# Anima-Lab/MaskDiT

Hardware: AMD Instinct MI355X
Metric: training img/sec MaskDiT-XL/2 256 mask=0.5 bs=1024 (higher is better)
Workload: dtype bf16; 1 GPU; DiT-XL/2 ImageNet256-latent [32x32x4], mask_ratio=0.5, mae_loss_coef=0.1, sample(moments)+class-dropout+fwd+bwd+grad-allreduce+AdamW+EMA, random-init (de-zeroed) weights; global_batch=1024, per_gpu_batch=1024, micro_batch=1024, accum=1, parallelism=dp1

## Files before the change

maskdit_amd/csrc/attention.hip:

```cpp
#include "common.h"
#include <type_traits>
#include "../../include/maskdit_hip.h"

template <int HD>
struct AttnCfg {
  static constexpr int HDK = (HD + 31) / 32 * 32;
  static constexpr int HDN = (HD + 15) / 16 * 16;
  static constexpr int KSTEPS = HDK / 32;
  static constexpr int NFRAG = HDN / 16;
  static constexpr int CH = HD / 8;
  static constexpr int PITCH_CH = (HDK / 8) | 1;
  static constexpr int PITCH = PITCH_CH * 16;
  static constexpr int TILE_BYTES = 64 * PITCH;
};

template <int HD> struct AttnRow {
  static constexpr int NFRAG = AttnCfg<HD>::NFRAG;
  static constexpr int NP = (NFRAG / 2 < HD / 32) ? NFRAG / 2 : HD / 32;
  static constexpr int NT = NFRAG - 2 * NP;
  uint4 pr[NP > 0 ? NP : 1];
  uint2 tl[NT > 0 ? NT : 1];
};
__device__ __forceinline__ unsigned attn_pack2(float a, float b) {
  bf16x2 t;
// ... 683 lines not shown
          for (int qi = 0; qi < QF; ++qi) s[qi][f] = mfma16(kfr, qf[qi][ks], s[qi][f]);
        }
      }
      bf16x8 pf[QF][KB / 32];
      if (kb + KB > Lv) {
#pragma unroll
        for (int qi = 0; qi < QF; ++qi)
#pragma unroll
          for (int f = 0; f < KB / 16; ++f)
#pragma unroll
            for (int r = 0; r < 4; ++r) s[qi][f][r] = (kb + 16 * f + 4 * g + r < Lv) ? s[qi][f][r] : -1e30f;
      }
#pragma unroll
      for (int qi = 0; qi < QF; ++qi) {
        float mx = -1e30f;
#pragma unroll
        for (int f = 0; f < KB / 16; ++f)
#pragma unroll
          for (int r = 0; r < 4; ++r) mx = fmaxf(mx, s[qi][f][r]);
        mx = group_max(mx);
        const float m_new = fmaxf(m_run[qi], mx * scale_log2e);
        const float alpha = fast_exp2(m_run[qi] - m_new);
        float psum = 0.f;
#pragma unroll
        for (int f = 0; f < KB / 16; ++f)
#pragma unroll
          for (int r = 0; r < 4; ++r) {
            const float pv = fast_exp2(__builtin_fmaf(s[qi][f][r], scale_log2e, -m_new));
            s[qi][f][r] = pv;
            psum += pv;
          }
        l_run[qi] = l_run[qi] * alpha + psum;
        m_run[qi] = m_new;
#pragma unroll
        for (int f = 0; f < C::NFRAG; ++f)
#pragma unroll
          for (int r = 0; r < 4; ++r) o[qi][f][r] *= alpha;
#pragma unroll
        for (int ks = 0; ks < KB / 32; ++ks) pf[qi][ks] = pack_pair(s[qi][2 * ks], s[qi][2 * ks + 1]);
      }
#pragma unroll
      for (int ks = 0; ks < KB / 32; ++ks)
#pragma unroll
        for (int f = 0; f < C::NFRAG; ++f) {
          const bf16x8 vfr = sp_frag_cols<HD, L>(Vs, kb + 32 * ks, f, i16, g);
#pragma unroll
          for (int qi = 0; qi < QF; ++qi) o[qi][f] = mfma16(vfr, pf[qi][ks], o[qi][f]);
        }
    }
#pragma unroll
    for (int qi = 0; qi < QF; ++qi) {
      const int q = wave * 16 * KF + 16 * (qp + qi) + i16;
      const float l_tot = group_sum(l_run[qi]);
      const float inv = 1.f / l_tot;
      bf16* orow = out + ((long)b * L + q) * D + h * HD;
      AttnRow<HD> orw;
      attn_pack_row<HD>(orw, o[qi], inv);
      attn_store_row<HD>(orow, g, orw);
      if (g == 0) lse[((long)b * H + h) * L + q] = m_run[qi] + log2f(l_tot);
    }
  }
}

__device__ __forceinline__ void sp_item_coords(int item, int B, int H, int& b, int& h) {
  const int full = (B >> 3) << 3;
  int sid;
  if (item < full * H) {
    const int xcd = item & 7, k = item >> 3;
    const int grp = k / H;
    sid = (grp * 8 + xcd) * H + (k - grp * H);
  } else {
    sid = item;
  }
  b = sid / H;
  h = sid - b * H;
}

#define SP_LDS_BARRIER()                                 \
  {                                                      \
    asm volatile("s_waitcnt lgkmcnt(0)" ::: "memory");   \
    __builtin_amdgcn_s_barrier();                        \
    asm volatile("" ::: "memory");                       \
  }
template <int HD, int KF, int OCC>
__global__ __launch_bounds__(512, OCC) void attn_bwd_sp_kernel(const bf16* __restrict__ qkv, const bf16* __restrict__ out,
                                                              const bf16* __restrict__ dout, const float* __restrict__ lse,
                                                              float* __restrict__ delta, bf16* __restrict__ dqkv, int H,
                                                              float scale, float scale_log2e, int Lv, int B, int dbg) {
  using C = SpCfg<HD>;
  constexpr int L = 128 * KF;
  constexpr int TILE = L * C::PITCH;
  __shared__ __attribute__((aligned(16))) char smem[4 * TILE + 2 * L * 4 + 64];
  char* Qs = smem;
  char* Ks = smem + TILE;
  char* Vs = smem + 2 * TILE;
  char* dOs = smem + 3 * TILE;
  float* lse_s = (float*)(smem + 4 * TILE);
  float* del_s = lse_s + L;
  const int tid = threadIdx.x, lane = tid & 63, wave = tid >> 6;
  const int i16 = lane & 15, g = lane >> 4;
  const int D = H * HD;
  const long ld = 3L * D;
  const int nitems = B * H;

  SpRegs<HD, L> r0, r1, r2, r3;
  bf16x8 of[KF][C::KSTEPS], dof[KF][C::KSTEPS];
  float lse_r = 0.f;
  auto fetch = [&](int item) {
    int b, h;
    sp_item_coords(item, B, H, b, h);
    const bf16* base = qkv + (long)b * L * ld + h * HD;
    const bf16* dobase = dout + (long)b * L * D + h * HD;
    const bf16* obase = out + (long)b * L * D + h * HD;
    sp_load_nb<HD, L>(r0, base, ld, tid);
    sp_load_nb<HD, L>(r1, base + D, ld, tid);
    sp_load_nb<HD, L>(r2, base + 2 * D, ld, tid);
    sp_load_nb<HD, L>(r3, dobase, D, tid);
    lse_r = lse[((long)b * H + h) * L + (tid & (L - 1))];
#pragma unroll
    for (int qi = 0; qi < KF; ++qi) {
      const int q = wave * 16 * KF + 16 * qi + i16;
#pragma unroll
      for (int s = 0; s < C::KSTEPS; ++s) {
        const int d = min(32 * s + 8 * g, HD - 8);
        of[qi][s] = *(const bf16x8*)(obase + (long)q * D + d);
        dof[qi][s] = *(const bf16x8*)(dobase + (long)q * D + d);
      }
    }
  };

  auto stage = [&](int it) {
    int b, h;
    sp_item_coords(it, B, H, b, h);
    const long bh = (long)b * H + h;
    sp_store<HD, L>(r0, Qs, tid);
    sp_store<HD, L>(r1, Ks, tid);
    sp_store<HD, L>(r2, Vs, tid);
    sp_store<HD, L>(r3, dOs, tid);
    if (tid < L) lse_s[tid] = lse_r;
#pragma unroll
    for (int qi = 0; qi < KF; ++qi) {
      const int q = wave * 16 * KF + 16 * qi + i16;
      float dl = 0.f;
#pragma unroll
      for (int s = 0; s < C::KSTEPS; ++s) {
        float part = 0.f;
#pragma unroll
        for (int e = 0; e < 8; ++e) part += bf2f(dof[qi][s][e]) * bf2f(of[qi][s][e]);
        dl += (32 * s + 8 * g < HD) ? part : 0.f;
      }
      dl = group_sum(dl);
      if (g == 0) {
        del_s[q] = dl * scale;
        delta[bh * L + q] = dl;
      }
    }
  };

  int item = blockIdx.x;
  if (item >= nitems) return;
  fetch(item);
  stage(item);
  for (;;) {
    int b, h;
    sp_item_coords(item, B, H, b, h);
    SP_LDS_BARRIER()
    const bool has_next = OCC == 2 && item + (int)gridDim.x < nitems;
    if (has_next && !MDT_EXP(dbg & 2)) fetch(item + gridDim.x);
    __builtin_amdgcn_sched_barrier(0);

#pragma unroll 1
    for (int ki = 0; ki < (MDT_EXP(dbg & 4) ? 0 : KF); ++ki) {
      const int k0 = wave * 16 * KF + 16 * ki;
      bf16x8 kf[C::KSTEPS], vf[C::KSTEPS];
#pragma unroll
      for (int ks = 0; ks < C::KSTEPS; ++ks) {
        kf[ks] = sp_frag_rows<HD, L>(Ks, k0 + i16, ks, g);
        vf[ks] = sp_frag_rows<HD, L>(Vs, k0 + i16, ks, g);
      }
      f32x4 dk[C::NFRAG], dv[C::NFRAG];
#pragma unroll
      for (int f = 0; f < C::NFRAG; ++f) {
        dk[f] = (f32x4){0.f, 0.f, 0.f, 0.f};
        dv[f] = (f32x4){0.f, 0.f, 0.f, 0.f};
      }
      const bool key_ok = (k0 + i16) < Lv;
#pragma unroll 1
      for (int qb = 0; qb < L; qb += 64) {
        f32x4 pm[4], ds[4];
#pragma unroll
        for (int f = 0; f < 4; ++f) {
          f32x4 s = (f32x4){0.f, 0.f, 0.f, 0.f}, dp = (f32x4){0.f, 0.f, 0.f, 0.f};
#pragma unroll
          for (int ks = 0; ks < C::KSTEPS; ++ks) {
            s = mfma16(sp_frag_rows<HD, L>(Qs, qb + 16 * f + i16, ks, g), kf[ks], s);
            dp = mfma16(sp_frag_rows<HD, L>(dOs, qb + 16 * f + i16, ks, g), vf[ks], dp);
          }
          const f32x4 ls = *(const f32x4*)(lse_s + qb + 16 * f + 4 * g);
          const f32x4 dl = *(const f32x4*)(del_s + qb + 16 * f + 4 * g);
#pragma unroll
          for (int r = 0; r < 4; ++r) {
            const float pv = fast_exp2(__builtin_fmaf(s[r], scale_log2e, -ls[r]));
            pm[f][r] = pv;
            ds[f][r] = pv * __builtin_fmaf(dp[r], scale, -dl[r]);
          }
        }
#pragma unroll
        for (int ks = 0; ks < 2; ++ks) {
          const bf16x8 pf = pack_pair(pm[2 * ks], pm[2 * ks + 1]);
          const bf16x8 dsf = pack_pair(ds[2 * ks], ds[2 * ks + 1]);
#pragma unroll
          for (int f = 0; f < C::NFRAG; ++f) {
            dv[f] = mfma16(sp_frag_cols<HD, L>(dOs, qb + 32 * ks, f, i16, g), pf, dv[f]);
            dk[f] = mfma16(sp_frag_cols<HD, L>(Qs, qb + 32 * ks, f, i16, g), dsf, dk[f]);
          }
        }
      }
      bf16* drow = dqkv + ((long)b * L + k0 + i16) * ld + h * HD;
      AttnRow<HD> krw, vrw;
      if (!key_ok) {
#pragma unroll
        for (int f = 0; f < C::NFRAG; ++f) dk[f] = dv[f] = (f32x4){0.f, 0.f, 0.f, 0.f};
      }
      attn_pack_row<HD>(krw, dk);
      attn_pack_row<HD>(vrw, dv);
      if (!MDT_EXP(dbg & 1)) {
        attn_store_row<HD>(drow + D, g, krw);
        attn_store_row<HD>(drow + 2 * D, g, vrw);
      }
    }

#pragma unroll 1
    for (int qi = 0; qi < (MDT_EXP(dbg & 8) ? 0 : KF); ++qi) {
      const int q = wave * 16 * KF + 16 * qi + i16;
      bf16x8 qf[C::KSTEPS], dqo[C::KSTEPS];
#pragma unroll
      for (int ks = 0; ks < C::KSTEPS; ++ks) {
        qf[ks] = sp_frag_rows<HD, L>(Qs, q, ks, g);
        dqo[ks] = sp_frag_rows<HD, L>(dOs, q, ks, g);
      }
      const float my_lse = lse_s[q], dl = del_s[q];
      f32x4 dq[C::NFRAG];
#pragma unroll
      for (int f = 0; f < C::NFRAG; ++f) dq[f] = (f32x4){0.f, 0.f, 0.f, 0.f};
#pragma unroll 1
      for (int kb = 0; kb < L; kb += 64) {
        f32x4 ds[4];
#pragma unroll
        for (int f = 0; f < 4; ++f) {
          f32x4 s = (f32x4){0.f, 0.f, 0.f, 0.f}, dp = (f32x4){0.f, 0.f, 0.f, 0.f};
#pragma unroll
          for (int ks = 0; ks < C::KSTEPS; ++ks) {
            s = mfma16(sp_frag_rows<HD, L>(Ks, kb + 16 * f + i16, ks, g), qf[ks], s);
            dp = mfma16(sp_frag_rows<HD, L>(Vs, kb + 16 * f + i16, ks, g), dqo[ks], dp);
          }
#pragma unroll
          for (int r = 0; r < 4; ++r) {
            const float pv = fast_exp2(__builtin_fmaf(s[r], scale_log2e, -my_lse));
            ds[f][r] = pv * __builtin_fmaf(dp[r], scale, -dl);
          }
        }
        if (kb + 64 > Lv) {
#pragma unroll
          for (int f = 0; f < 4; ++f)
#pragma unroll
            for (int r = 0; r < 4; ++r) ds[f][r] = (kb + 16 * f + 4 * g + r < Lv) ? ds[f][r] : 0.f;
        }
#pragma unroll
        for (int ks = 0; ks < 2; ++ks) {
          const bf16x8 dsf = pack_pair(ds[2 * ks], ds[2 * ks + 1]);
#pragma unroll
          for (int f = 0; f < C::NFRAG; ++f) dq[f] = mfma16(sp_frag_cols<HD, L>(Ks, kb + 32 * ks, f, i16, g), dsf, dq[f]);
        }
      }
      bf16* drow = dqkv + ((long)b * L + q) * ld + h * HD;
      AttnRow<HD> qrw;
      attn_pack_row<HD>(qrw, dq);
      if (!MDT_EXP(dbg & 1)) attn_store_row<HD>(drow, g, qrw);
    }
    if (!has_next) break;
    SP_LDS_BARRIER()
    item += gridDim.x;
    stage(item);
  }
}

template <int HD>
__device__ __forceinline__ void attn_bwd_item_math(const char* Qs, const char* Ks, const char* Vs, const char* dOs,
                                                   const float* lse_s, const float* del_s, bf16* dbase, long ld, int D,
                                                   int wave, int i16, int g, int Lv, float scale, float scale_log2e,
                                                   AttnRow<HD>& q_cur, const AttnRow<HD>& q_prev) {
  using C = SpCfg<HD>;
  constexpr int L = 128;
  AttnRow<HD> k_keep, v_keep;
  {
    const int k0 = wave * 16;
    bf16x8 kf[C::KSTEPS], vf[C::KSTEPS];
#pragma unroll
    for (int ks = 0; ks < C::KSTEPS; ++ks) {
      kf[ks] = sp_frag_rows<HD, L>(Ks, k0 + i16, ks, g);
      vf[ks] = sp_frag_rows<HD, L>(Vs, k0 + i16, ks, g);
    }
    f32x4 dk[C::NFRAG], dv[C::NFRAG];
#pragma unroll
    for (int f = 0; f < C::NFRAG; ++f) {
      dk[f] = (f32x4){0.f, 0.f, 0.f, 0.f};
      dv[f] = (f32x4){0.f, 0.f, 0.f, 0.f};
    }
    const bool key_ok = (k0 + i16) < Lv;
#pragma unroll 1
    for (int qb = 0; qb < L; qb += 64) {
      f32x4 pm[4], ds[4];
#pragma unroll
      for (int f = 0; f < 4; ++f) {
        f32x4 s = (f32x4){0.f, 0.f, 0.f, 0.f}, dp = (f32x4){0.f, 0.f, 0.f, 0.f};
#pragma unroll
        for (int ks = 0; ks < C::KSTEPS; ++ks) {
          s = mfma16(sp_frag_rows<HD, L>(Qs, qb + 16 * f + i16, ks, g), kf[ks], s);
          dp = mfma16(sp_frag_rows<HD, L>(dOs, qb + 16 * f + i16, ks, g), vf[ks], dp);
        }
        const f32x4 ls = *(const f32x4*)(lse_s + qb + 16 * f + 4 * g);
        const f32x4 dl = *(const f32x4*)(del_s + qb + 16 * f + 4 * g);
#pragma unroll
        for (int r = 0; r < 4; ++r) {
          const float pv = fast_exp2(__builtin_fmaf(s[r], scale_log2e, -ls[r]));
          pm[f][r] = pv;
          ds[f][r] = pv * __builtin_fmaf(dp[r], scale, -dl[r]);
        }
      }
#pragma unroll
      for (int ks = 0; ks < 2; ++ks) {
        const bf16x8 pf = pack_pair(pm[2 * ks], pm[2 * ks + 1]);
        const bf16x8 dsf = pack_pair(ds[2 * ks], ds[2 * ks + 1]);
#pragma unroll
        for (int f = 0; f < C::NFRAG; ++f) {
          dv[f] = mfma16(sp_frag_cols<HD, L>(dOs, qb + 32 * ks, f, i16, g), pf, dv[f]);
          dk[f] = mfma16(sp_frag_cols<HD, L>(Qs, qb + 32 * ks, f, i16, g), dsf, dk[f]);
        }
      }
    }
    bf16* drow = dbase + (long)(k0 + i16) * ld;
    if (!key_ok) {
#pragma unroll
      for (int f = 0; f < C::NFRAG; ++f) dk[f] = dv[f] = (f32x4){0.f, 0.f, 0.f, 0.f};
    }
    attn_pack_row<HD>(k_keep, dk);
    attn_pack_row<HD>(v_keep, dv);
    attn_store_row<HD>(drow + D, g, k_keep);
    attn_store_row<HD>(drow + 2 * D, g, v_keep);
    attn_keep_alive<HD>(q_prev);
  }
  {
    const int q = wave * 16 + i16;
    bf16x8 qf[C::KSTEPS], dqo[C::KSTEPS];
#pragma unroll
    for (int ks = 0; ks < C::KSTEPS; ++ks) {
      qf[ks] = sp_frag_rows<HD, L>(Qs, q, ks, g);
      dqo[ks] = sp_frag_rows<HD, L>(dOs, q, ks, g);
    }
    const float my_lse = lse_s[q], dl = del_s[q];
    f32x4 dq[C::NFRAG];
#pragma unroll
    for (int f = 0; f < C::NFRAG; ++f) dq[f] = (f32x4){0.f, 0.f, 0.f, 0.f};
#pragma unroll 1
    for (int kb = 0; kb < L; kb += 64) {
      f32x4 ds[4];
#pragma unroll
      for (int f = 0; f < 4; ++f) {
        f32x4 s = (f32x4){0.f, 0.f, 0.f, 0.f}, dp = (f32x4){0.f, 0.f, 0.f, 0.f};
#pragma unroll
        for (int ks = 0; ks < C::KSTEPS; ++ks) {
          s = mfma16(sp_frag_rows<HD, L>(Ks, kb + 16 * f + i16, ks, g), qf[ks], s);
          dp = mfma16(sp_frag_rows<HD, L>(Vs, kb + 16 * f + i16, ks, g), dqo[ks], dp);
        }
#pragma unroll
        for (int r = 0; r < 4; ++r) {
          const float pv = fast_exp2(__builtin_fmaf(s[r], scale_log2e, -my_lse));
          ds[f][r] = pv * __builtin_fmaf(dp[r], scale, -dl);
        }
      }
      if (kb + 64 > Lv) {
#pragma unroll
        for (int f = 0; f < 4; ++f)
#pragma unroll
          for (int r = 0; r < 4; ++r) ds[f][r] = (kb + 16 * f + 4 * g + r < Lv) ? ds[f][r] : 0.f;
      }
#pragma unroll
      for (int ks = 0; ks < 2; ++ks) {
        const bf16x8 dsf = pack_pair(ds[2 * ks], ds[2 * ks + 1]);
#pragma unroll
        for (int f = 0; f < C::NFRAG; ++f) dq[f] = mfma16(sp_frag_cols<HD, L>(Ks, kb + 32 * ks, f, i16, g), dsf, dq[f]);
      }
    }
    bf16* drow = dbase + (long)q * ld;
    attn_pack_row<HD>(q_cur, dq);
    attn_store_row<HD>(drow, g, q_cur);
    attn_keep_alive<HD>(k_keep);
    attn_keep_alive<HD>(v_keep);
  }
}

template <int HD>
__global__ __launch_bounds__(512, 2) void attn_bwd_dma_kernel(const bf16* __restrict__ qkv, const bf16* __restrict__ out,
                                                               const bf16* __restrict__ dout, const float* __restrict__ lse,
                                                               float* __restrict__ delta, bf16* __restrict__ dqkv, int H,
                                                               float scale, float scale_log2e, int Lv, int B) {
  using C = SpCfg<HD>;
  static_assert(C::PITCH == HD * 2, "tile rows must be contiguous in LDS (odd chunk count)");
  constexpr int L = 128;
  constexpr int TILE = L * C::PITCH;
  constexpr int HALF_CH = L * C::CH / 2;
  static_assert(HALF_CH % 64 == 0, "a wave moves whole 1-KiB pieces");
  constexpr int NDMA = HALF_CH / 64;
  constexpr int NSTORE = 1 + 3 * (AttnRow<HD>::NP + AttnRow<HD>::NT);
  __shared__ __attribute__((aligned(16))) char buf0[4 * TILE];
  __shared__ __attribute__((aligned(16))) char buf1[4 * TILE];
  __shared__ float lse_s0[L], lse_s1[L], del_s[L];
  const int tid = threadIdx.x, lane = tid & 63;
  const int wave = __builtin_amdgcn_readfirstlane(tid >> 6);
  const int i16 = lane & 15, g = lane >> 4;
  const int D = H * HD;
  const long ld = 3L * D;
  const int nitems = B * H;

  static_assert(NDMA == 9, "nine 1-KiB pieces per wave");
  const int tw = wave >> 1, hw = wave & 1;
  const long row_bytes = (tw < 3 ? ld : (long)D) * 2;
  unsigned doff[NDMA];
  int lds_main, lds_tail;
  if constexpr (sp_split<HD, L>) {
#pragma unroll
    for (int j = 0; j < 8; ++j) {
      const int r = 64 * hw + 8 * j + (lane >> 3), c = (lane & 7) ^ (lane >> 3);
      doff[j] = (unsigned)(r * row_bytes + c * 16);
    }
    doff[8] = (unsigned)((64 * hw + lane) * row_bytes + 128);
    lds_main = tw * TILE + hw * 8192;
    lds_tail = tw * TILE + L * 128 + hw * 1024;
  } else {
#pragma unroll
    for (int j = 0; j < NDMA; ++j) {
      const int idx = hw * HALF_CH + 64 * j + lane;
      const int r = idx / C::CH, c = idx - r * C::CH;
      doff[j] = (unsigned)(r * row_bytes + c * 16);
    }
    lds_main = tw * TILE + hw * HALF_CH * 16;
    lds_tail = lds_main + 8192;
  }
  auto item_src = [&](int item) -> const char* {
    int b, h;
    sp_item_coords(item, B, H, b, h);
    return tw < 3 ? (const char*)(qkv + (long)b * L * ld + h * HD + tw * D) : (const char*)(dout + (long)b * L * D + h * HD);
  };

  float lse_r = 0.f;
  bf16x8 of0[C::KSTEPS], of1[C::KSTEPS];
  AttnRow<HD> qk0, qk1;
#pragma unroll
  for (int q = 0; q < (AttnRow<HD>::NP > 0 ? AttnRow<HD>::NP : 1); ++q) qk0.pr[q] = qk1.pr[q] = make_uint4(0u, 0u, 0u, 0u);
#pragma unroll
  for (int t = 0; t < (AttnRow<HD>::NT > 0 ? AttnRow<HD>::NT : 1); ++t) qk0.tl[t] = qk1.tl[t] = make_uint2(0u, 0u);
  const int qrow = wave * 16 + i16;

#define ATTN_DMA_BARRIER()                                                                    \
  {                                                                                           \
    asm volatile("s_waitcnt lgkmcnt(0)" ::: "memory");                                        \
    __builtin_amdgcn_s_barrier();                                                             \
    asm volatile("" ::: "memory");                                                            \
  }
#define ATTN_DMA_BODY(P, CUR, NXT, LSE_CUR, LSE_NXT, OF_CUR, OF_NXT, QK_CUR, QK_PRV, VMWAIT)                             \
  {                                                                                                        \
    int b, h;                                                                                              \
    sp_item_coords(item, B, H, b, h);                                                                      \
    const long bh = (long)b * H + h;                                                                       \
    const char* Qs = CUR;                                                                                  \
    const char* Ks = CUR + TILE;                                                                           \
    const char* Vs = CUR + 2 * TILE;                                                                       \
    const char* dOs = CUR + 3 * TILE;                                                                      \
                                                                        \
    asm volatile("; MDT_CHK hand_wait" ::: "memory");                                                      \
    __builtin_amdgcn_s_waitcnt(((VMWAIT) & 15) | (7 << 4) | (15 << 8) | (((VMWAIT) >> 4) << 14));  \
    asm volatile("" ::: "memory");                                                                         \
    if (tid < L) LSE_CUR[tid] = lse_r;                                                                     \
    asm volatile("; MDT_CHK no_dma" ::: "memory");  \
    ATTN_DMA_BARRIER()                \
    const int nxt = item + (int)gridDim.x;                                                                 \
    {       \
      const int fit = nxt < nitems ? nxt : item;                                                           \
      const char* src = item_src(fit);                                                                     \
      _Pragma("unroll") for (int j = 0; j < 8; ++j) glds16(src + opaque(doff[j]), NXT + lds_main + 1024 * j); \
      glds16(src + opaque(doff[8]), NXT + lds_tail);                                                       \
      int nb, nh;                                                                                          \
      sp_item_coords(fit, B, H, nb, nh);                                                                   \
      lse_r = lse[((long)nb * H + nh) * L + (tid & (L - 1))];                                              \
      const bf16* orow = out + ((long)nb * L + qrow) * D + nh * HD;                                        \
      _Pragma("unroll") for (int s2 = 0; s2 < C::KSTEPS; ++s2)                                             \
        OF_NXT[s2] = *(const bf16x8*)(orow + min(32 * s2 + 8 * g, HD - 8));                                \
    }                                                                                                      \
    __builtin_amdgcn_sched_barrier(0);                                                                     \
    {                                                   \
      float dl = 0.f;                                                                                      \
      _Pragma("unroll") for (int s2 = 0; s2 < C::KSTEPS; ++s2) {                                           \
        const bf16x8 dof = sp_frag_rows<HD, L>(dOs, qrow, s2, g);                                             \
        float part = 0.f;                                                                                  \
        _Pragma("unroll") for (int e = 0; e < 8; ++e) part += bf2f(dof[e]) * bf2f(OF_CUR[s2][e]);          \
        dl += (32 * s2 + 8 * g < HD) ? part : 0.f;                                                         \
      }                                                                                                    \
      dl = group_sum(dl);                                                                                  \
      if (g == 0) {                                                                                        \
        del_s[qrow] = dl * scale;              \
        delta[bh * L + qrow] = dl;                                                                         \
      }                                                                                                    \
    }                                                                                                      \
    ATTN_DMA_BARRIER()                                               \
    attn_bwd_item_math<HD>(Qs, Ks, Vs, dOs, LSE_CUR, del_s, dqkv + (long)b * L * ld + h * HD, ld, D, wave, i16, g, Lv, \
                           scale, scale_log2e, QK_CUR, QK_PRV);                                            \
    item = nxt;                                                                                            \
  }

  int item = blockIdx.x;
  if (item >= nitems) return;
  {
    const char* src = item_src(item);
#pragma unroll
    for (int j = 0; j < 8; ++j) glds16(src + opaque(doff[j]), buf0 + lds_main + 1024 * j);
    glds16(src + opaque(doff[8]), buf0 + lds_tail);
    int b, h;
    sp_item_coords(item, B, H, b, h);
    lse_r = lse[((long)b * H + h) * L + (tid & (L - 1))];
    const bf16* orow = out + ((long)b * L + qrow) * D + h * HD;
#pragma unroll
    for (int s2 = 0; s2 < C::KSTEPS; ++s2) of0[s2] = *(const bf16x8*)(orow + min(32 * s2 + 8 * g, HD - 8));
#pragma unroll
    for (int s2 = 0; s2 < C::KSTEPS; ++s2) of1[s2] = of0[s2];
  }
#ifdef MDT_REGRESS_R3_ATTN_WAIT
  ATTN_DMA_BODY(0, buf0, buf1, lse_s0, lse_s1, of0, of1, qk0, qk1, NSTORE)
#else
  ATTN_DMA_BODY(0, buf0, buf1, lse_s0, lse_s1, of0, of1, qk0, qk1, 0)
#endif
  while (item < nitems) {
    ATTN_DMA_BODY(1, buf1, buf0, lse_s1, lse_s0, of1, of0, qk1, qk0, NSTORE)
    if (item >= nitems) break;
    ATTN_DMA_BODY(0, buf0, buf1, lse_s0, lse_s1, of0, of1, qk0, qk1, NSTORE)
  }
#undef ATTN_DMA_BODY
#undef ATTN_DMA_BARRIER
}

template <int HD, int KF>
__global__ __launch_bounds__(512, 2) void attn_bwd_q_res_kernel(const bf16* __restrict__ qkv, const bf16* __restrict__ out,
                                                                 const bf16* __restrict__ dout, const float* __restrict__ lse,
                                                                 float* __restrict__ delta, bf16* __restrict__ dqkv, int H,
                                                                 float scale, float scale_log2e, int Lv) {
  using C = SpCfg<HD>;
  constexpr int L = 128 * KF;
  constexpr int TILE = L * sp_pitch<HD, L>;
  __shared__ __attribute__((aligned(16))) char smem[2 * TILE + 64];
  char* Ks = smem;
  char* Vs = smem + TILE;
  const int tid = threadIdx.x, lane = tid & 63, wave = tid >> 6;
  const int i16 = lane & 15, g = lane >> 4;
  int b, h;
  sp_block_coords(gridDim.y / H, H, b, h);
  const long bh = (long)b * H + h;
  const int D = H * HD;
  const long ld = 3L * D;
  const bf16* base = qkv + (long)b * L * ld + h * HD;
  {
    SpRegs<HD, L> kreg, vreg;
    sp_load_nb<HD, L>(kreg, base + D, ld, tid);
    sp_load_nb<HD, L>(vreg, base + 2 * D, ld, tid);
    sp_store<HD, L>(kreg, Ks, tid);
    sp_store<HD, L>(vreg, Vs, tid);
  }
  __syncthreads();
#pragma unroll 1
  for (int qi = 0; qi < KF; ++qi) {
    const int q = wave * 16 * KF + 16 * qi + i16;
    const long orow = ((long)b * L + q) * D + h * HD;
    bf16x8 qf[C::KSTEPS], dqo[C::KSTEPS], of[C::KSTEPS];
#pragma unroll
    for (int s2 = 0; s2 < C::KSTEPS; ++s2) {
      const int d = min(32 * s2 + 8 * g, HD - 8);
      qf[s2] = *(const bf16x8*)(base + (long)q * ld + d);
      dqo[s2] = *(const bf16x8*)(dout + orow + d);
      of[s2] = *(const bf16x8*)(out + orow + d);
    }
    const float my_lse = lse[bh * L + q];
    float dl = 0.f;
#pragma unroll
    for (int s2 = 0; s2 < C::KSTEPS; ++s2) {
      const bool in = 32 * s2 + 8 * g < HD;
      float part = 0.f;
#pragma unroll
      for (int e = 0; e < 8; ++e) {
        part += bf2f(dqo[s2][e]) * bf2f(of[s2][e]);
        qf[s2][e] = in ? qf[s2][e] : (bf16)0.f;
        dqo[s2][e] = in ? dqo[s2][e] : (bf16)0.f;
      }
      dl += in ? part : 0.f;
    }
    dl = group_sum(dl);
    if (g == 0) delta[bh * L + q] = dl;
    const float dl_s = dl * scale;
    f32x4 dq[C::NFRAG];
#pragma unroll
    for (int f = 0; f < C::NFRAG; ++f) dq[f] = (f32x4){0.f, 0.f, 0.f, 0.f};
#pragma unroll 1
    for (int kb = 0; kb < L; kb += 64) {
      f32x4 ds[4];
#pragma unroll
      for (int f = 0; f < 4; ++f) {
        f32x4 sv = (f32x4){0.f, 0.f, 0.f, 0.f}, dp = (f32x4){0.f, 0.f, 0.f, 0.f};
#pragma unroll
        for (int ks = 0; ks < C::KSTEPS; ++ks) {
          sv = mfma16(sp_frag_rows<HD, L>(Ks, kb + 16 * f + i16, ks, g), qf[ks], sv);
          dp = mfma16(sp_frag_rows<HD, L>(Vs, kb + 16 * f + i16, ks, g), dqo[ks], dp);
        }
#pragma unroll
        for (int r = 0; r < 4; ++r) {
          const float pv = fast_exp2(__builtin_fmaf(sv[r], scale_log2e, -my_lse));
          ds[f][r] = pv * __builtin_fmaf(dp[r], scale, -dl_s);
        }
      }
      if (kb + 64 > Lv) {
#pragma unroll
        for (int f = 0; f < 4; ++f)
#pragma unroll
          for (int r = 0; r < 4; ++r) ds[f][r] = (kb + 16 * f + 4 * g + r < Lv) ? ds[f][r] : 0.f;
// ... 107 lines not shown
        for (int f = 0; f < C::NFRAG; ++f) {
          dv[f] = mfma16(sp_frag_cols<HD, L>(dOs, qb + 32 * ks, f, i16, g), pf, dv[f]);
          dk[f] = mfma16(sp_frag_cols<HD, L>(Qs, qb + 32 * ks, f, i16, g), dsf, dk[f]);
        }
      }
    }
    bf16* drow = dqkv + ((long)b * L + k0 + i16) * ld + h * HD;
    AttnRow<HD> krw, vrw;
    if (key_pen != 0.f) {
#pragma unroll
      for (int f = 0; f < C::NFRAG; ++f) dk[f] = dv[f] = (f32x4){0.f, 0.f, 0.f, 0.f};
    }
    attn_pack_row<HD>(krw, dk);
    attn_pack_row<HD>(vrw, dv);
    attn_store_row<HD>(drow + D, g, krw);
    attn_store_row<HD>(drow + 2 * D, g, vrw);
  }
}


#define ATTN_DISPATCH(HD_, CALL) \
  switch (HD_) {                 \
    case 32: { constexpr int HDc = 32; CALL; } break; \
    case 64: { constexpr int HDc = 64; CALL; } break; \
    case 72: { constexpr int HDc = 72; CALL; } break; \
    case 80: { constexpr int HDc = 80; CALL; } break; \
    default: mdt_set_error("attention: head_dim must be one of 32, 64, 72, 80"); return MDT_ERR_ARG; \
  }

int nt8_num_cus();
static int attn_num_cus() { return nt8_num_cus() & ~7; }

extern "C" int mdt_attn_fwd(const mdt_bf16* qkv, mdt_bf16* out, float* lse, int B, int L, int H, int hd, int L_valid,
                            mdt_stream_t stream) {
  MDT_REQUIRE(qkv && out && lse, "attn_fwd: null pointer");
  MDT_REQUIRE(B > 0 && H > 0 && L > 0 && L % 64 == 0, "attn_fwd: L must be a positive multiple of 64");
  if (L_valid <= 0 || L_valid > L) L_valid = L;
  float sl = (1.0f / sqrtf((float)hd)) * 1.4426950408889634f;
  if ((L == 128 || L == 256) && mdt_get_tuning_int(MDT_TUNE_ATTN_SP) != 1) {
    dim3 grid(1, B * H);
    const bool pad = L_valid < L;
    if (L == 128 && !pad) {
      ATTN_DISPATCH(hd, hipLaunchKernelGGL((attn_fwd_sp_kernel<HDc, 1, false>), grid, dim3(512), 0, (hipStream_t)stream,
                                           (const bf16*)qkv, (bf16*)out, lse, H, sl, L_valid));
    } else if (L == 128) {
      ATTN_DISPATCH(hd, hipLaunchKernelGGL((attn_fwd_sp_kernel<HDc, 1, true>), grid, dim3(512), 0, (hipStream_t)stream,
                                           (const bf16*)qkv, (bf16*)out, lse, H, sl, L_valid));
    } else if (!pad) {
      ATTN_DISPATCH(hd, hipLaunchKernelGGL((attn_fwd_sp_kernel<HDc, 2, false>), grid, dim3(512), 0, (hipStream_t)stream,
                                           (const bf16*)qkv, (bf16*)out, lse, H, sl, L_valid));
    } else {
      ATTN_DISPATCH(hd, hipLaunchKernelGGL((attn_fwd_sp_kernel<HDc, 2, true>), grid, dim3(512), 0, (hipStream_t)stream,
                                           (const bf16*)qkv, (bf16*)out, lse, H, sl, L_valid));
    }
    return mdt_check_launch("attn_fwd_sp");
  }
  if (L == 512 && hd == 72 && mdt_get_tuning_int(MDT_TUNE_ATTN_SP) != 1) {
    if (L_valid < L)
      hipLaunchKernelGGL((attn_fwd_sp_kernel<72, 4, true>), dim3(1, B * H), dim3(512), 0, (hipStream_t)stream, (const bf16*)qkv,
                         (bf16*)out, lse, H, sl, L_valid);
    else
      hipLaunchKernelGGL((attn_fwd_sp_kernel<72, 4, false>), dim3(1, B * H), dim3(512), 0, (hipStream_t)stream, (const bf16*)qkv,
                         (bf16*)out, lse, H, sl, L_valid);
    return mdt_check_launch("attn_fwd_sp");
  }
  if (L == 1024 && hd == 32 && mdt_get_tuning_int(MDT_TUNE_ATTN_SP) != 1) {
    hipLaunchKernelGGL((attn_fwd_res_kernel<32, 8>), dim3(1, B * H), dim3(512), 0, (hipStream_t)stream, (const bf16*)qkv,
                       (bf16*)out, lse, H, sl, L_valid);
    return mdt_check_launch("attn_fwd_res");
  }
  const int qf_knob = mdt_get_tuning_int(MDT_TUNE_ATTN_QF);
  if (L % 128 == 0 && (qf_knob == 2 || (qf_knob == 0 && hd <= 64))) {
    dim3 grid(L / 128, B * H);
    ATTN_DISPATCH(hd, hipLaunchKernelGGL((attn_fwd_kernel<HDc, 2>), grid, dim3(256), 0, (hipStream_t)stream,
                                         (const bf16*)qkv, (bf16*)out, lse, L, H, sl, L_valid));
  } else {
    dim3 grid(L / 64, B * H);
    ATTN_DISPATCH(hd, hipLaunchKernelGGL((attn_fwd_kernel<HDc, 1>), grid, dim3(256), 0, (hipStream_t)stream,
                                         (const bf16*)qkv, (bf16*)out, lse, L, H, sl, L_valid));
  }
  return mdt_check_launch("attn_fwd");
}

extern "C" int mdt_attn_bwd(const mdt_bf16* qkv, const mdt_bf16* out, const mdt_bf16* dout, const float* lse,
                            float* delta, mdt_bf16* dqkv, int B, int L, int H, int hd, int L_valid,
                            mdt_stream_t stream) {
  MDT_REQUIRE(qkv && out && dout && lse && delta && dqkv, "attn_bwd: null pointer");
  MDT_REQUIRE(B > 0 && H > 0 && L > 0 && L % 64 == 0, "attn_bwd: L must be a positive multiple of 64");
  if (L_valid <= 0 || L_valid > L) L_valid = L;
  float sc = 1.0f / sqrtf((float)hd);
  float sl = sc * 1.4426950408889634f;
  const int sp_knob = mdt_get_tuning_int(MDT_TUNE_ATTN_SP);
  const int adbg = MDT_EXP(1) ? mdt_get_tuning_int(MDT_TUNE_ATTN_DBG) : 0;
  const bool sp_ok = L == 128 || (L == 256 && (hd == 32 || hd == 64 || hd == 72));
  if (sp_ok && sp_knob != 1 && (L == 128 || hd <= 64 || sp_knob == 2)) {
    dim3 g1(B * H);
    const int items = B * H;
    const int cus = attn_num_cus();
    dim3 gp(items < cus ? items : cus);
    if (L == 128 && hd == 72 && sp_knob != 2 && sp_knob != 3) {
      hipLaunchKernelGGL(attn_bwd_dma_kernel<72>, gp, dim3(512), 0, (hipStream_t)stream, (const bf16*)qkv, (const bf16*)out,
                         (const bf16*)dout, lse, delta, (bf16*)dqkv, H, sc, sl, L_valid, B);
    } else if (L == 128 && sp_knob == 2) {
      ATTN_DISPATCH(hd, hipLaunchKernelGGL((attn_bwd_sp_kernel<HDc, 1, 4>), g1, dim3(512), 0, (hipStream_t)stream,
                                           (const bf16*)qkv, (const bf16*)out, (const bf16*)dout, lse, delta, (bf16*)dqkv, H,
                                           sc, sl, L_valid, B, adbg));
    } else if (L == 128) {
      ATTN_DISPATCH(hd, hipLaunchKernelGGL((attn_bwd_sp_kernel<HDc, 1, 2>), gp, dim3(512), 0, (hipStream_t)stream,
                                           (const bf16*)qkv, (const bf16*)out, (const bf16*)dout, lse, delta, (bf16*)dqkv, H,
                                           sc, sl, L_valid, B, adbg));
    } else {
      switch (hd) {
        case 32: hipLaunchKernelGGL((attn_bwd_sp_kernel<32, 2, 2>), gp, dim3(512), 0, (hipStream_t)stream, (const bf16*)qkv,
                                    (const bf16*)out, (const bf16*)dout, lse, delta, (bf16*)dqkv, H, sc, sl, L_valid, B, adbg); break;
        case 64: hipLaunchKernelGGL((attn_bwd_sp_kernel<64, 2, 2>), gp, dim3(512), 0, (hipStream_t)stream, (const bf16*)qkv,
                                    (const bf16*)out, (const bf16*)dout, lse, delta, (bf16*)dqkv, H, sc, sl, L_valid, B, adbg); break;
        default: hipLaunchKernelGGL((attn_bwd_sp_kernel<72, 2, 2>), gp, dim3(512), 0, (hipStream_t)stream, (const bf16*)qkv,
                                    (const bf16*)out, (const bf16*)dout, lse, delta, (bf16*)dqkv, H, sc, sl, L_valid, B, adbg); break;
      }
    }
    return mdt_check_launch("attn_bwd_sp");
  }
  if (L == 512 && hd == 72 && sp_knob != 1) {
    hipLaunchKernelGGL((attn_bwd_q_res_kernel<72, 4>), dim3(1, B * H), dim3(512), 0, (hipStream_t)stream, (const bf16*)qkv,
                       (const bf16*)out, (const bf16*)dout, lse, delta, (bf16*)dqkv, H, sc, sl, L_valid);
    int rc = mdt_check_launch("attn_bwd_q_res");
    if (rc) return rc;
    hipLaunchKernelGGL((attn_bwd_kv_res_kernel<72, 4>), dim3(1, B * H), dim3(512), 0, (hipStream_t)stream, (const bf16*)qkv,
                       (const bf16*)dout, lse, delta, (bf16*)dqkv, H, sc, sl, L_valid);
    return mdt_check_launch("attn_bwd_kv_res");
  }
  if (L == 1024 && hd == 32 && sp_knob != 1) {
    hipLaunchKernelGGL((attn_bwd_q_res_kernel<32, 8>), dim3(1, B * H), dim3(512), 0, (hipStream_t)stream, (const bf16*)qkv,
                       (const bf16*)out, (const bf16*)dout, lse, delta, (bf16*)dqkv, H, sc, sl, L_valid);
    int rc = mdt_check_launch("attn_bwd_q_res");
    if (rc) return rc;
    hipLaunchKernelGGL((attn_bwd_kv_res_kernel<32, 8>), dim3(1, B * H), dim3(512), 0, (hipStream_t)stream, (const bf16*)qkv,
                       (const bf16*)dout, lse, delta, (bf16*)dqkv, H, sc, sl, L_valid);
    return mdt_check_launch("attn_bwd_kv_res");
  }
  dim3 grid(L / 64, B * H);
  ATTN_DISPATCH(hd, hipLaunchKernelGGL(attn_bwd_dq_kernel<HDc>, grid, dim3(256), 0, (hipStream_t)stream,
                                       (const bf16*)qkv, (const bf16*)out, (const bf16*)dout, lse, delta,
                                       (bf16*)dqkv, L, H, sc, sl, L_valid));
  int rc = mdt_check_launch("attn_bwd_dq");
  if (rc) return rc;
  ATTN_DISPATCH(hd, hipLaunchKernelGGL(attn_bwd_dkv_kernel<HDc>, grid, dim3(256), 0, (hipStream_t)stream,
                                       (const bf16*)qkv, (const bf16*)dout, lse, delta, (bf16*)dqkv, L, H, sc, sl, L_valid));
  return mdt_check_launch("attn_bwd_dkv");
}
```

Measured before the change: 2283 img/s.

## Compute attention backward dQ in one pass from dS staged in LDS

```diff
diff --git a/maskdit_amd/csrc/attention.hip b/maskdit_amd/csrc/attention.hip
--- a/maskdit_amd/csrc/attention.hip
+++ b/maskdit_amd/csrc/attention.hip
@@ -789,7 +789,21 @@
     __builtin_amdgcn_s_barrier();                        \
     asm volatile("" ::: "memory");                       \
   }
-template <int HD, int KF, int OCC>
+template <int L> constexpr int ds_pitch = 2 * L + 32;
+template <int L>
+__device__ __forceinline__ void ds_stage(char* img, int key, int q0, int g, bf16x8 dsf, bool key_ok) {
+  const uint4 v = __builtin_bit_cast(uint4, dsf);
+  char* p = img + key * ds_pitch<L> + (q0 + 4 * g) * 2;
+  *(uint2*)p = make_uint2(key_ok ? v.x : 0u, key_ok ? v.y : 0u);
+  *(uint2*)(p + 32) = make_uint2(key_ok ? v.z : 0u, key_ok ? v.w : 0u);
+}
+template <int L>
+__device__ __forceinline__ bf16x8 ds_frag_cols(const char* img, int rbase, int fd, int i16, int g) {
+  const char* q = img + (rbase + 4 * g + (i16 >> 2)) * ds_pitch<L> + (16 * fd + 4 * (i16 & 3)) * 2;
+  return cat4(lds_tr_read(q), lds_tr_read(q + 16 * ds_pitch<L>));
+}
+
+template <int HD, int KF, int OCC, bool ONEPASS = false>
 __global__ __launch_bounds__(512, OCC) void attn_bwd_sp_kernel(const bf16* __restrict__ qkv, const bf16* __restrict__ out,
                                                               const bf16* __restrict__ dout, const float* __restrict__ lse,
                                                               float* __restrict__ delta, bf16* __restrict__ dqkv, int H,
@@ -797,7 +811,10 @@
   using C = SpCfg<HD>;
   constexpr int L = 128 * KF;
   constexpr int TILE = L * C::PITCH;
-  __shared__ __attribute__((aligned(16))) char smem[4 * TILE + 2 * L * 4 + 64];
+  static_assert(!ONEPASS || (OCC == 2 && !sp_swz4<HD, L> && !sp_split<HD, L>), "one-pass form: plain-pitch tiles, one workgroup per CU");
+  constexpr int DS_OFF = (4 * TILE + 2 * L * 4 + 64 + 15) & ~15;
+  __shared__ __attribute__((aligned(16))) char smem[ONEPASS ? DS_OFF + 128 * ds_pitch<L> : 4 * TILE + 2 * L * 4 + 64];
+  char* dSs = smem + (ONEPASS ? DS_OFF : 0);
   char* Qs = smem;
   char* Ks = smem + TILE;
   char* Vs = smem + 2 * TILE;
@@ -876,6 +893,12 @@
     if (has_next && !MDT_EXP(dbg & 2)) fetch(item + gridDim.x);
     __builtin_amdgcn_sched_barrier(0);
 
+    f32x4 dq1[KF][C::NFRAG];
+#pragma unroll
+    for (int qi = 0; qi < KF; ++qi)
+#pragma unroll
+      for (int f = 0; f < C::NFRAG; ++f) dq1[qi][f] = (f32x4){0.f, 0.f, 0.f, 0.f};
+
 #pragma unroll 1
     for (int ki = 0; ki < (MDT_EXP(dbg & 4) ? 0 : KF); ++ki) {
       const int k0 = wave * 16 * KF + 16 * ki;
@@ -916,6 +939,7 @@
         for (int ks = 0; ks < 2; ++ks) {
           const bf16x8 pf = pack_pair(pm[2 * ks], pm[2 * ks + 1]);
           const bf16x8 dsf = pack_pair(ds[2 * ks], ds[2 * ks + 1]);
+          if constexpr (ONEPASS) ds_stage<L>(dSs, 16 * wave + i16, qb + 32 * ks, g, dsf, key_ok);
 #pragma unroll
           for (int f = 0; f < C::NFRAG; ++f) {
             dv[f] = mfma16(sp_frag_cols<HD, L>(dOs, qb + 32 * ks, f, i16, g), pf, dv[f]);
@@ -935,10 +959,38 @@
         attn_store_row<HD>(drow + D, g, krw);
         attn_store_row<HD>(drow + 2 * D, g, vrw);
       }
+      if constexpr (ONEPASS) {
+        SP_LDS_BARRIER()
+        if (!MDT_EXP(dbg & 8)) {
+#pragma unroll
+          for (int ks = 0; ks < 4; ++ks) {
+            bf16x8 dst[KF];
+#pragma unroll
+            for (int qi = 0; qi < KF; ++qi) dst[qi] = ds_frag_cols<L>(dSs, 32 * ks, wave * KF + qi, i16, g);
+#pragma unroll
+            for (int f = 0; f < C::NFRAG; ++f) {
+              const char* kq = Ks + (32 * KF * ks + 16 * ki + 4 * g + (i16 >> 2)) * C::PITCH + (16 * f + 4 * (i16 & 3)) * 2;
+              const bf16x8 kt = cat4(lds_tr_read(kq), lds_tr_read(kq + 16 * KF * C::PITCH));
+#pragma unroll
+              for (int qi = 0; qi < KF; ++qi) dq1[qi][f] = mfma16(kt, dst[qi], dq1[qi][f]);
+            }
+          }
+        }
+        if (ki + 1 < KF) SP_LDS_BARRIER()
+      }
+    }
+    if constexpr (ONEPASS) {
+#pragma unroll
+      for (int qi = 0; qi < KF; ++qi) {
+        bf16* drow = dqkv + ((long)b * L + wave * 16 * KF + 16 * qi + i16) * ld + h * HD;
+        AttnRow<HD> qrw;
+        attn_pack_row<HD>(qrw, dq1[qi]);
+        if (!MDT_EXP(dbg & 1)) attn_store_row<HD>(drow, g, qrw);
+      }
     }
 
 #pragma unroll 1
-    for (int qi = 0; qi < (MDT_EXP(dbg & 8) ? 0 : KF); ++qi) {
+    for (int qi = 0; qi < (ONEPASS || MDT_EXP(dbg & 8) ? 0 : KF); ++qi) {
       const int q = wave * 16 * KF + 16 * qi + i16;
       bf16x8 qf[C::KSTEPS], dqo[C::KSTEPS];
 #pragma unroll
@@ -992,7 +1044,7 @@
   }
 }
 
-template <int HD>
+template <int HD, bool ONEPASS>
 __device__ __forceinline__ void attn_bwd_item_math(const char* Qs, const char* Ks, const char* Vs, const char* dOs,
                                                    const float* lse_s, const float* del_s, bf16* dbase, long ld, int D,
                                                    int wave, int i16, int g, int Lv, float scale, float scale_log2e,
@@ -1015,8 +1067,8 @@
       dv[f] = (f32x4){0.f, 0.f, 0.f, 0.f};
     }
     const bool key_ok = (k0 + i16) < Lv;
-#pragma unroll 1
-    for (int qb = 0; qb < L; qb += 64) {
+    bf16x8 dsk[ONEPASS ? L / 32 : 1];
+    auto phase_a = [&](int qb, bf16x8* keep) {
       f32x4 pm[4], ds[4];
 #pragma unroll
       for (int f = 0; f < 4; ++f) {
@@ -1039,12 +1091,24 @@
       for (int ks = 0; ks < 2; ++ks) {
         const bf16x8 pf = pack_pair(pm[2 * ks], pm[2 * ks + 1]);
         const bf16x8 dsf = pack_pair(ds[2 * ks], ds[2 * ks + 1]);
+        if constexpr (ONEPASS) keep[ks] = dsf;
 #pragma unroll
         for (int f = 0; f < C::NFRAG; ++f) {
           dv[f] = mfma16(sp_frag_cols<HD, L>(dOs, qb + 32 * ks, f, i16, g), pf, dv[f]);
           dk[f] = mfma16(sp_frag_cols<HD, L>(Qs, qb + 32 * ks, f, i16, g), dsf, dk[f]);
         }
       }
+    };
+    if constexpr (ONEPASS) {
+#pragma unroll
+      for (int qb = 0; qb < L; qb += 64) phase_a(qb, dsk + qb / 32);
+      SP_LDS_BARRIER()
+      char* img = const_cast<char*>(Vs);
+#pragma unroll
+      for (int j = 0; j < L / 32; ++j) ds_stage<L>(img, k0 + i16, 32 * j, g, dsk[j], key_ok);
+    } else {
+#pragma unroll 1
+      for (int qb = 0; qb < L; qb += 64) phase_a(qb, dsk);
     }
     bf16* drow = dbase + (long)(k0 + i16) * ld;
     if (!key_ok) {
@@ -1057,61 +1121,79 @@
     attn_store_row<HD>(drow + 2 * D, g, v_keep);
     attn_keep_alive<HD>(q_prev);
   }
-  {
+  if constexpr (ONEPASS) {
+    static_assert(128 * ds_pitch<L> <= 2 * L * C::PITCH, "the dS image must fit the V and dO tiles");
     const int q = wave * 16 + i16;
-    bf16x8 qf[C::KSTEPS], dqo[C::KSTEPS];
-#pragma unroll
-    for (int ks = 0; ks < C::KSTEPS; ++ks) {
-      qf[ks] = sp_frag_rows<HD, L>(Qs, q, ks, g);
-      dqo[ks] = sp_frag_rows<HD, L>(dOs, q, ks, g);
-    }
-    const float my_lse = lse_s[q], dl = del_s[q];
     f32x4 dq[C::NFRAG];
 #pragma unroll
     for (int f = 0; f < C::NFRAG; ++f) dq[f] = (f32x4){0.f, 0.f, 0.f, 0.f};
-#pragma unroll 1
-    for (int kb = 0; kb < L; kb += 64) {
-      f32x4 ds[4];
-#pragma unroll
-      for (int f = 0; f < 4; ++f) {
-        f32x4 s = (f32x4){0.f, 0.f, 0.f, 0.f}, dp = (f32x4){0.f, 0.f, 0.f, 0.f};
-#pragma unroll
-        for (int ks = 0; ks < C::KSTEPS; ++ks) {
-          s = mfma16(sp_frag_rows<HD, L>(Ks, kb + 16 * f + i16, ks, g), qf[ks], s);
-          dp = mfma16(sp_frag_rows<HD, L>(Vs, kb + 16 * f + i16, ks, g), dqo[ks], dp);
-        }
-#pragma unroll
-        for (int r = 0; r < 4; ++r) {
-          const float pv = fast_exp2(__builtin_fmaf(s[r], scale_log2e, -my_lse));
-          ds[f][r] = pv * __builtin_fmaf(dp[r], scale, -dl);
-        }
-      }
-      if (kb + 64 > Lv) {
-#pragma unroll
-        for (int f = 0; f < 4; ++f)
-#pragma unroll
-          for (int r = 0; r < 4; ++r) ds[f][r] = (kb + 16 * f + 4 * g + r < Lv) ? ds[f][r] : 0.f;
-      }
-#pragma unroll
-      for (int ks = 0; ks < 2; ++ks) {
-        const bf16x8 dsf = pack_pair(ds[2 * ks], ds[2 * ks + 1]);
-#pragma unroll
-        for (int f = 0; f < C::NFRAG; ++f) dq[f] = mfma16(sp_frag_cols<HD, L>(Ks, kb + 32 * ks, f, i16, g), dsf, dq[f]);
-      }
+    SP_LDS_BARRIER()
+#pragma unroll
+    for (int ks = 0; ks < L / 32; ++ks) {
+      const bf16x8 dst = ds_frag_cols<L>(Vs, 32 * ks, wave, i16, g);
+#pragma unroll
+      for (int f = 0; f < C::NFRAG; ++f) dq[f] = mfma16(sp_frag_cols<HD, L>(Ks, 32 * ks, f, i16, g), dst, dq[f]);
     }
     bf16* drow = dbase + (long)q * ld;
     attn_pack_row<HD>(q_cur, dq);
     attn_store_row<HD>(drow, g, q_cur);
     attn_keep_alive<HD>(k_keep);
     attn_keep_alive<HD>(v_keep);
-  }
-}
-
-template <int HD>
-__global__ __launch_bounds__(512, 2) void attn_bwd_dma_kernel(const bf16* __restrict__ qkv, const bf16* __restrict__ out,
-                                                               const bf16* __restrict__ dout, const float* __restrict__ lse,
-                                                               float* __restrict__ delta, bf16* __restrict__ dqkv, int H,
-                                                               float scale, float scale_log2e, int Lv, int B) {
+  } else {
+    const int q = wave * 16 + i16;
+    bf16x8 qf[C::KSTEPS], dqo[C::KSTEPS];
+#pragma unroll
+    for (int ks = 0; ks < C::KSTEPS; ++ks) {
+      qf[ks] = sp_frag_rows<HD, L>(Qs, q, ks, g);
+      dqo[ks] = sp_frag_rows<HD, L>(dOs, q, ks, g);
+    }
+    const float my_lse = lse_s[q], dl = del_s[q];
+    f32x4 dq[C::NFRAG];
+#pragma unroll
+    for (int f = 0; f < C::NFRAG; ++f) dq[f] = (f32x4){0.f, 0.f, 0.f, 0.f};
+#pragma unroll 1
+    for (int kb = 0; kb < L; kb += 64) {
+      f32x4 ds[4];
+#pragma unroll
+      for (int f = 0; f < 4; ++f) {
+        f32x4 s = (f32x4){0.f, 0.f, 0.f, 0.f}, dp = (f32x4){0.f, 0.f, 0.f, 0.f};
+#pragma unroll
+        for (int ks = 0; ks < C::KSTEPS; ++ks) {
+          s = mfma16(sp_frag_rows<HD, L>(Ks, kb + 16 * f + i16, ks, g), qf[ks], s);
+          dp = mfma16(sp_frag_rows<HD, L>(Vs, kb + 16 * f + i16, ks, g), dqo[ks], dp);
+        }
+#pragma unroll
+        for (int r = 0; r < 4; ++r) {
+          const float pv = fast_exp2(__builtin_fmaf(s[r], scale_log2e, -my_lse));
+          ds[f][r] = pv * __builtin_fmaf(dp[r], scale, -dl);
+        }
+      }
+      if (kb + 64 > Lv) {
+#pragma unroll
+        for (int f = 0; f < 4; ++f)
+#pragma unroll
+          for (int r = 0; r < 4; ++r) ds[f][r] = (kb + 16 * f + 4 * g + r < Lv) ? ds[f][r] : 0.f;
+      }
+#pragma unroll
+      for (int ks = 0; ks < 2; ++ks) {
+        const bf16x8 dsf = pack_pair(ds[2 * ks], ds[2 * ks + 1]);
+#pragma unroll
+        for (int f = 0; f < C::NFRAG; ++f) dq[f] = mfma16(sp_frag_cols<HD, L>(Ks, kb + 32 * ks, f, i16, g), dsf, dq[f]);
+      }
+    }
+    bf16* drow = dbase + (long)q * ld;
+    attn_pack_row<HD>(q_cur, dq);
+    attn_store_row<HD>(drow, g, q_cur);
+    attn_keep_alive<HD>(k_keep);
+    attn_keep_alive<HD>(v_keep);
+  }
+}
+
+template <int HD, bool ONEPASS, bool R3WAIT>
+__device__ __forceinline__ void attn_bwd_dma_impl(const bf16* __restrict__ qkv, const bf16* __restrict__ out,
+                                                  const bf16* __restrict__ dout, const float* __restrict__ lse,
+                                                  float* __restrict__ delta, bf16* __restrict__ dqkv, int H,
+                                                  float scale, float scale_log2e, int Lv, int B) {
   using C = SpCfg<HD>;
   static_assert(C::PITCH == HD * 2, "tile rows must be contiguous in LDS (odd chunk count)");
   constexpr int L = 128;
@@ -1191,6 +1273,8 @@
     if (tid < L) LSE_CUR[tid] = lse_r;                                                                     \
     asm volatile("; MDT_CHK no_dma" ::: "memory");  \
     ATTN_DMA_BARRIER()                \
+                            \
+    _Pragma("unroll") for (int s2 = 0; s2 < C::KSTEPS; ++s2) asm volatile("" ::"v"(OF_CUR[s2]));           \
     const int nxt = item + (int)gridDim.x;                                                                 \
     {       \
       const int fit = nxt < nitems ? nxt : item;                                                           \
@@ -1220,7 +1304,7 @@
       }                                                                                                    \
     }                                                                                                      \
     ATTN_DMA_BARRIER()                                               \
-    attn_bwd_item_math<HD>(Qs, Ks, Vs, dOs, LSE_CUR, del_s, dqkv + (long)b * L * ld + h * HD, ld, D, wave, i16, g, Lv, \
+    attn_bwd_item_math<HD, ONEPASS>(Qs, Ks, Vs, dOs, LSE_CUR, del_s, dqkv + (long)b * L * ld + h * HD, ld, D, wave, i16, g, Lv, \
                            scale, scale_log2e, QK_CUR, QK_PRV);                                            \
     item = nxt;                                                                                            \
   }
@@ -1241,11 +1325,7 @@
 #pragma unroll
     for (int s2 = 0; s2 < C::KSTEPS; ++s2) of1[s2] = of0[s2];
   }
-#ifdef MDT_REGRESS_R3_ATTN_WAIT
-  ATTN_DMA_BODY(0, buf0, buf1, lse_s0, lse_s1, of0, of1, qk0, qk1, NSTORE)
-#else
-  ATTN_DMA_BODY(0, buf0, buf1, lse_s0, lse_s1, of0, of1, qk0, qk1, 0)
-#endif
+  ATTN_DMA_BODY(0, buf0, buf1, lse_s0, lse_s1, of0, of1, qk0, qk1, (R3WAIT ? NSTORE : 0))
   while (item < nitems) {
     ATTN_DMA_BODY(1, buf1, buf0, lse_s1, lse_s0, of1, of0, qk1, qk0, NSTORE)
     if (item >= nitems) break;
@@ -1253,6 +1333,27 @@
   }
 #undef ATTN_DMA_BODY
 #undef ATTN_DMA_BARRIER
+}
+
+constexpr bool ATTN_ENC_ONEPASS = true;
+#ifdef MDT_REGRESS_R3_ATTN_WAIT
+constexpr bool ATTN_R3WAIT = true;
+#else
+constexpr bool ATTN_R3WAIT = false;
+#endif
+template <int HD>
+__global__ __launch_bounds__(512, 2) void attn_bwd_dma_kernel(const bf16* __restrict__ qkv, const bf16* __restrict__ out,
+                                                               const bf16* __restrict__ dout, const float* __restrict__ lse,
+                                                               float* __restrict__ delta, bf16* __restrict__ dqkv, int H,
+                                                               float scale, float scale_log2e, int Lv, int B) {
+  attn_bwd_dma_impl<HD, ATTN_ENC_ONEPASS, ATTN_R3WAIT>(qkv, out, dout, lse, delta, dqkv, H, scale, scale_log2e, Lv, B);
+}
+template <int HD>
+__global__ __launch_bounds__(512, 2) void attn_bwd_dma_kernel_2p(const bf16* __restrict__ qkv, const bf16* __restrict__ out,
+                                                                  const bf16* __restrict__ dout, const float* __restrict__ lse,
+                                                                  float* __restrict__ delta, bf16* __restrict__ dqkv, int H,
+                                                                  float scale, float scale_log2e, int Lv, int B) {
+  attn_bwd_dma_impl<HD, false, false>(qkv, out, dout, lse, delta, dqkv, H, scale, scale_log2e, Lv, B);
 }
 
 template <int HD, int KF>
@@ -1526,6 +1627,8 @@
   return mdt_check_launch("attn_fwd");
 }
 
+constexpr bool ATTN_DEC_ONEPASS = !sp_swz4<32, 256>;
+
 extern "C" int mdt_attn_bwd(const mdt_bf16* qkv, const mdt_bf16* out, const mdt_bf16* dout, const float* lse,
                             float* delta, mdt_bf16* dqkv, int B, int L, int H, int hd, int L_valid,
                             mdt_stream_t stream) {
@@ -1543,8 +1646,12 @@
     const int cus = attn_num_cus();
     dim3 gp(items < cus ? items : cus);
     if (L == 128 && hd == 72 && sp_knob != 2 && sp_knob != 3) {
-      hipLaunchKernelGGL(attn_bwd_dma_kernel<72>, gp, dim3(512), 0, (hipStream_t)stream, (const bf16*)qkv, (const bf16*)out,
-                         (const bf16*)dout, lse, delta, (bf16*)dqkv, H, sc, sl, L_valid, B);
+      if (sp_knob == 4 && ATTN_ENC_ONEPASS)
+        hipLaunchKernelGGL(attn_bwd_dma_kernel_2p<72>, gp, dim3(512), 0, (hipStream_t)stream, (const bf16*)qkv,
+                           (const bf16*)out, (const bf16*)dout, lse, delta, (bf16*)dqkv, H, sc, sl, L_valid, B);
+      else
+        hipLaunchKernelGGL(attn_bwd_dma_kernel<72>, gp, dim3(512), 0, (hipStream_t)stream, (const bf16*)qkv,
+                           (const bf16*)out, (const bf16*)dout, lse, delta, (bf16*)dqkv, H, sc, sl, L_valid, B);
     } else if (L == 128 && sp_knob == 2) {
       ATTN_DISPATCH(hd, hipLaunchKernelGGL((attn_bwd_sp_kernel<HDc, 1, 4>), g1, dim3(512), 0, (hipStream_t)stream,
                                            (const bf16*)qkv, (const bf16*)out, (const bf16*)dout, lse, delta, (bf16*)dqkv, H,
@@ -1555,8 +1662,15 @@
                                            sc, sl, L_valid, B, adbg));
     } else {
       switch (hd) {
-        case 32: hipLaunchKernelGGL((attn_bwd_sp_kernel<32, 2, 2>), gp, dim3(512), 0, (hipStream_t)stream, (const bf16*)qkv,
-                                    (const bf16*)out, (const bf16*)dout, lse, delta, (bf16*)dqkv, H, sc, sl, L_valid, B, adbg); break;
+        case 32:
+          if (sp_knob == 4)
+            hipLaunchKernelGGL((attn_bwd_sp_kernel<32, 2, 2>), gp, dim3(512), 0, (hipStream_t)stream, (const bf16*)qkv,
+                               (const bf16*)out, (const bf16*)dout, lse, delta, (bf16*)dqkv, H, sc, sl, L_valid, B, adbg);
+          else
+            hipLaunchKernelGGL((attn_bwd_sp_kernel<32, 2, 2, ATTN_DEC_ONEPASS>), gp, dim3(512), 0, (hipStream_t)stream,
+                               (const bf16*)qkv, (const bf16*)out, (const bf16*)dout, lse, delta, (bf16*)dqkv, H, sc, sl, L_valid,
+                               B, adbg);
+          break;
         case 64: hipLaunchKernelGGL((attn_bwd_sp_kernel<64, 2, 2>), gp, dim3(512), 0, (hipStream_t)stream, (const bf16*)qkv,
                                     (const bf16*)out, (const bf16*)dout, lse, delta, (bf16*)dqkv, H, sc, sl, L_valid, B, adbg); break;
         default: hipLaunchKernelGGL((attn_bwd_sp_kernel<72, 2, 2>), gp, dim3(512), 0, (hipStream_t)stream, (const bf16*)qkv,
```

After: 2295 img/s (median of 6 runs). No clear change (+0.5%).
